# bacpop/ska.rust

Hardware: AMD Instinct MI355X
Metric: genomes/sec ska build+align, 1 000x5 Mbp k=31; bit-exact vs CPU (higher is better)
Workload: dtype u64

## Files before the change

### ska.rust_amd/csrc/skx_api.cpp

```cpp
#include "skx_internal.h"
#include "../../include/skx_host.h"
#include <algorithm>
#include <atomic>
#include <chrono>
#include <cmath>
#include <cstdarg>
#include <cstddef>
#include <cstdio>
#include <cstring>
#include <map>
#include <memory>
#include <mutex>
#include <numeric>
#include <optional>
#include <unordered_map>
#include <thread>
#include <cerrno>
#include <fcntl.h>
#include <sys/mman.h>
#include <sys/stat.h>
#include <unistd.h>

using namespace skx;

// ... 1115 lines not shown
    }
    SKX_HIP(hipStreamSynchronize(st));
    *out = a.release();
    return SKX_OK;
}
static int lazy_check_missing(skx_array *a, DevBuf<int> &d_flag)
{
    int missing = 0;
    SKX_HIP(hipMemcpyAsync(&missing, d_flag.p, 4, hipMemcpyDeviceToHost, a->ctx->stream));
    SKX_HIP(hipStreamSynchronize(a->ctx->stream));
    SKX_HIP(hipGetLastError());
    if (missing) { set_error("row keyset does not contain every split k-mer of the samples"); return SKX_EINVAL; }
    return SKX_OK;
}
extern "C" int skx_array_assemble_lazy(skx_ctx *ctx, skx_dictset *d, skx_keyset *rows, const char *const *names, skx_array **out)
{
    return skx_guarded([&]() -> int {
    if (!ctx || !d || !rows || !out) { skx_dictset_free(d); skx_keyset_free(rows); set_error("bad arguments"); return SKX_EINVAL; }
    if (rows->holds_pieces_of(d)) {
        const int r = skx_array_assemble(ctx, d, rows, names, out);
        skx_dictset_free(d); skx_keyset_free(rows);
        return r;
    }
    if (rows->wide != d->wide() || rows->k != d->k || rows->rc != d->rc || rows->logN < 0 || rows->logN < d->logB || d->n > 65535 || knob("eager_array")) {
        const int r = skx_array_assemble(ctx, d, rows, names, out);
        skx_dictset_free(d); skx_keyset_free(rows);
        return r;
    }
    SKX_HIP(hipSetDevice(ctx->device));
    { const int rs = dictset_sort(d); if (rs != SKX_OK) { skx_dictset_free(d); skx_keyset_free(rows); return rs; } }
    return array_make_lazy(ctx, d, rows, names, out);
    });
}
static int pieces_stats_pass(skx_array *a, uint64_t min_count)
{
    skx_ctx *ctx = a->ctx; hipStream_t st = ctx->stream;
    const skx_pieces *pc = a->pieces; const skx_keyset *blk = a->lazy_rows;
    const int S = (int)a->names.size(), nb = 1 << pc->logQ;
    ctx->cut_ranks = ctx->cut_blocks = 0;
    if (!a->n_rows) return SKX_OK;
    const uint32_t stage = min_count >= 2 ? pieces_stats_bound(pc->cap) : 0u;
    DevBuf<uint32_t> r_cut; DevBuf<unsigned long long> tally;
    if (stage) { SKX_TRY(r_cut.alloc((size_t)nb)); SKX_TRY(tally.alloc(2)); SKX_TRY(tally.zero(st)); }
    unsigned long long h_tally[2] = {0, 0};
    {
        StageTimer t(ctx, &ctx->tm.assemble);
        KernelTimer kt(ctx, &ctx->tm.pieces_stats);
        if (stage) launch_pieces_cut(pc->plen.p, S, pc->cap, (uint32_t)std::min<uint64_t>(min_count, 0xFFFFFFFEull), pc->nrank.p, blk->ncnt.p, stage, nb, r_cut.p, tally.p, st);
        launch_pieces_stats(pc->data.p, pc->plen.p, pc->perm.p, pc->nrank.p, blk->ncnt.p, blk->roff.p, pc->cap, S, nb, a->present.p, a->unambig.p, a->mask.p, a->vcount.p, st,
                            stage ? r_cut.p : nullptr);
        if (stage) SKX_HIP(hipMemcpyAsync(h_tally, tally.p, 16, hipMemcpyDeviceToHost, st));
    }
    SKX_HIP(hipStreamSynchronize(st));
    SKX_HIP(hipGetLastError());
    ctx->cut_ranks = h_tally[0]; ctx->cut_blocks = h_tally[1];
    if (stage && getenv("SKX_DEBUG")) fprintf(stderr, "[skx] filter: min_count %llu, the rank bound left %llu ranks unread over %llu of %d row blocks\n", (unsigned long long)min_count, h_tally[0], h_tally[1], nb);
    return SKX_OK;
}
int skx::array_lazy_stats(skx_array *a)
{
    if (!a->lazy() || a->stats_ready) return SKX_OK;
    skx_ctx *ctx = a->ctx; hipStream_t st = ctx->stream;
    SKX_HIP(hipSetDevice(ctx->device));
    if (a->pieces) {
        SKX_TRY(pieces_stats_pass(a, 0));
        a->stats_ready = true;
        return SKX_OK;
    }
    DevBuf<int> d_flag; SKX_TRY(d_flag.alloc(1)); SKX_TRY(d_flag.zero(st));
    if (a->n_rows) {
        AssembleArgs aa = lazy_args(a, d_flag.p);
        { StageTimer t(ctx, &ctx->tm.assemble); launch_assemble_lazy(a, aa, st, 1); }
        SKX_HIP(hipMemcpyAsync(a->vcount.p, a->present.p, a->n_rows * 4, hipMemcpyDeviceToDevice, st));
    }
    SKX_TRY(lazy_check_missing(a, d_flag));
    a->stats_ready = true;
    return SKX_OK;
}
int skx::array_materialize(skx_array *a)
{
    if (!a->lazy()) return SKX_OK;
    skx_ctx *ctx = a->ctx; hipStream_t st = ctx->stream;
    SKX_HIP(hipSetDevice(ctx->device));
    if (a->pieces) SKX_TRY(array_lazy_stats(a));
    const uint64_t U = a->n_rows; const size_t S = a->names.size();
    a->pitch = pitch_for(U);
    SKX_TRY(a->matrix.alloc((uint64_t)S * a->pitch));
    DevBuf<int> d_flag; SKX_TRY(d_flag.alloc(1)); SKX_TRY(d_flag.zero(st));
    if (a->pieces) {
// ... 560 lines not shown
                launch_compact_u64(a->keys.p, k2.p, U, keep.p, pos.p, st);
                a->keys = std::move(k2);
            } else if (a->host_keys.empty()) {
                DevBuf<uint64_t> k2; SKX_TRY(k2.alloc(kept * 2));
                launch_compact_u128(a->keys.p, k2.p, U, keep.p, pos.p, st);
                a->keys = std::move(k2);
            } else {
                std::vector<uint8_t> hkeep(U);
                SKX_HIP(hipMemcpyAsync(hkeep.data(), keep.p, U, hipMemcpyDeviceToHost, st));
                SKX_HIP(hipStreamSynchronize(st));
                std::vector<skx_key> nk; nk.reserve(kept);
                for (uint64_t i = 0; i < U; i++) if (hkeep[i] == 1) nk.push_back(a->host_keys[i]);
                a->host_keys.swap(nk);
            }
            a->n_kmers = kept;
        }
        SKX_HIP(hipStreamSynchronize(st));
        a->matrix = std::move(nm); a->present = std::move(p2); a->unambig = std::move(u2); a->mask = std::move(m2); a->vcount = std::move(v2);
        a->pitch = np; a->n_rows = kept;
        a->drop_lazy();
        a->stats_ready = true;
    }
    return SKX_OK;
}

extern "C" int skx_array_filter(skx_array *a, uint64_t min_count, int filter_ambig_as_missing, int filter_type, int mask_ambig,
                                int ignore_const_gaps, int update_kmers, int32_t *removed)
{
    return skx_guarded([&]() -> int {
    skx_ctx *ctx = a->ctx; hipStream_t st = ctx->stream;
    SKX_HIP(hipSetDevice(ctx->device));
    const uint64_t U = a->n_rows; const size_t S = a->names.size();
    ctx->cut_ranks = ctx->cut_blocks = 0;
    if (a->pieces && !a->stats_ready && !filter_ambig_as_missing && min_count >= 2 && a->total_samples == 0 && !knob("stats_eager"))
        SKX_TRY(pieces_stats_pass(a, min_count));
    else
        SKX_TRY(array_lazy_stats(a));
    DevBuf<uint8_t> keep; DevBuf<uint64_t> pos;
    SKX_TRY(keep.alloc(U)); SKX_TRY(pos.alloc(U + 1));
    uint64_t kept = 0, silent = 0;
    {
        StageTimer t(ctx, &ctx->tm.filter);
        FilterArgs fa{a->vcount.p, a->present.p, a->unambig.p, a->mask.p, U, (uint32_t)(a->total_samples ? a->total_samples : S), min_count, filter_ambig_as_missing, filter_type, ignore_const_gaps, keep.p};
        launch_filter_flags(fa, st);
        DevBuf<uint32_t> sc_sums; DevBuf<uint64_t> sc_offs;
        SKX_TRY(sc_sums.alloc(scan_u8_blocks(U))); SKX_TRY(sc_offs.alloc(scan_u8_blocks(U) + 1));
        launch_scan_u8(keep.p, pos.p, U, sc_sums.p, sc_offs.p, st);
        SKX_HIP(hipMemcpyAsync(&kept, pos.p + U, 8, hipMemcpyDeviceToHost, st));
        if (filter_ambig_as_missing) {
            DevBuf<unsigned long long> d_sil; SKX_TRY(d_sil.alloc(1)); SKX_TRY(d_sil.zero(st));
            launch_count_u8(keep.p, U, 2, d_sil.p, st);
            unsigned long long s2 = 0;
            SKX_HIP(hipMemcpyAsync(&s2, d_sil.p, 8, hipMemcpyDeviceToHost, st));
            SKX_HIP(hipStreamSynchronize(st));
            silent = s2;
        }
        SKX_HIP(hipStreamSynchronize(st));
    }
    SKX_TRY(array_compact(a, keep, pos, kept, mask_ambig, filter_ambig_as_missing != 0, update_kmers || filter_ambig_as_missing));
    SKX_HIP(hipGetLastError());
    if (removed) *removed = (int32_t)(U - kept - silent);
    return SKX_OK;
    });
}


static int array_keep_rows(skx_array *a, DevBuf<uint8_t> &keep, uint64_t *removed)
{
    hipStream_t st = a->ctx->stream;
    const uint64_t U = a->n_rows;
    DevBuf<uint64_t> pos; SKX_TRY(pos.alloc(U + 1));
    uint64_t kept = 0;
    DevBuf<uint32_t> sc_sums; DevBuf<uint64_t> sc_offs;
    SKX_TRY(sc_sums.alloc(scan_u8_blocks(U))); SKX_TRY(sc_offs.alloc(scan_u8_blocks(U) + 1));
    launch_scan_u8(keep.p, pos.p, U, sc_sums.p, sc_offs.p, st);
    SKX_HIP(hipMemcpyAsync(&kept, pos.p + U, 8, hipMemcpyDeviceToHost, st));
    SKX_HIP(hipStreamSynchronize(st));
    SKX_TRY(array_compact(a, keep, pos, kept, 0, false, true));
    SKX_HIP(hipGetLastError());
    if (removed) *removed = U - kept;
    return SKX_OK;
}

extern "C" skx_ctx *skx_array_ctx(const skx_array *a) { return a->ctx; }
extern "C" void skx_set_last_error(const char *msg) { set_error("%s", msg ? msg : ""); }

extern "C" int skx_keyset_from_fasta(skx_ctx *ctx, const char *path, int k, int rc, skx_keyset **out)
{
    return skx_guarded([&]() -> int {
    if (!ctx || !path || !out) { set_error("bad arguments"); return SKX_EINVAL; }
    SKX_TRY(check_k(k));
// ... 335 lines not shown
```

### ska.rust_amd/csrc/skx_append.hip

```cpp
#include "skx_device.h"
#include <cstdlib>
#include <type_traits>

namespace skx {

typedef uint32_t u32x4 __attribute__((ext_vector_type(4)));
typedef const u32x4 __attribute__((address_space(1))) *g4_t;

#ifdef SKX_AP_PROF
__device__ unsigned long long g_ap_prof[16];
#define AP_PROF_START unsigned long long tprof = __builtin_readcyclecounter(), tacc[12] = {0, 0, 0, 0, 0, 0, 0, 0, 0, 0, 0, 0}
#define AP_PROF(i) do { const unsigned long long t_ = __builtin_readcyclecounter(); tacc[(i)] += t_ - tprof; tprof = t_; } while (0)
#define AP_PROF_FLUSH() do { for (int i_ = 0; i_ < 12; i_++) if (tacc[i_] && (i_ >= 6 || (threadIdx.x & 63) == 0)) atomicAdd(&g_ap_prof[i_], tacc[i_]); } while (0)
extern "C" void skx_debug_phase_prof(unsigned long long *out, int reset)
{
    unsigned long long h[16];
    (void)hipDeviceSynchronize();
    (void)hipMemcpyFromSymbol(h, HIP_SYMBOL(g_ap_prof), sizeof(h));
    for (int i = 0; i < 16; i++) out[i] = h[i];
    if (reset) { for (auto &x : h) x = 0; (void)hipMemcpyToSymbol(HIP_SYMBOL(g_ap_prof), h, sizeof(h)); }
}
#else
#define AP_PROF_START do { } while (0)
#define AP_PROF(i) do { } while (0)
// ... 426 lines not shown
        }
    }
    __syncthreads();
    uint16_t *pj = a.perm + j * (uint64_t)cap;
    for (uint32_t i = tid; i < cap; i += AP_THREADS) pj[i] = s_perm[i];
    if (tid == 0) { a.ncnt[j] = total; a.nrank[j] = nr < cap ? nr : cap; if (total > a.stride) atomicOr(a.overflow, 1); }
    __syncthreads();
    }
}

template <bool COUNT_ONLY>
static void launch_append_t(const AppendArgs &a, unsigned blocks, hipStream_t st)
{
    const size_t lds = append_lds_bytes(a.nslots, a.cap, COUNT_ONLY);
    const bool hi = a.bits - a.logQ >= 32;
    if (hi) {
        (void)hipFuncSetAttribute((const void *)append_kernel<COUNT_ONLY, true>, hipFuncAttributeMaxDynamicSharedMemorySize, (int)lds);
        hipLaunchKernelGGL((append_kernel<COUNT_ONLY, true>), dim3(blocks), dim3(AP_THREADS), lds, st, a);
    } else {
        (void)hipFuncSetAttribute((const void *)append_kernel<COUNT_ONLY, false>, hipFuncAttributeMaxDynamicSharedMemorySize, (int)lds);
        hipLaunchKernelGGL((append_kernel<COUNT_ONLY, false>), dim3(blocks), dim3(AP_THREADS), lds, st, a);
    }
}
bool append_ok(int bits, int logB, int logQ, uint32_t region_cap, uint32_t nslots, uint32_t cap)
{
    const int rem = bits - logQ;
    (void)region_cap;
    return logQ >= logB && rem >= 0 && rem <= 50 && cap % 128u == 0 && cap >= 128u && cap <= APPEND_MAX_CAP && nslots >= cap && (nslots & (nslots - 1u)) == 0u &&
           append_lds_bytes(nslots, cap, false) <= 160u * 1024u - 256u;
}
void launch_append(const AppendArgs &a, uint32_t region_cap, hipStream_t st) { (void)region_cap; launch_append_t<false>(a, (1u << a.logQ) / a.rounds, st); }
void launch_append_probe(const AppendArgs &a, uint32_t region_cap, unsigned blocks, hipStream_t st) { (void)region_cap; launch_append_t<true>(a, blocks, st); }

__global__ __launch_bounds__(256) void pieces_cut_kernel(const uint16_t *plen, int S, uint32_t cap, uint32_t min_count, const uint32_t *nrank, const uint32_t *ncnt,
                                                         uint32_t stage, uint32_t *r_cut, unsigned long long *tally)
{
    extern __shared__ uint32_t s_hist[];
    __shared__ uint32_t s_sum[256];
    __shared__ uint32_t s_cut;
    const uint64_t j = blockIdx.x;
    const uint32_t tid = threadIdx.x, nbin = cap + 1u, share = (nbin + 255u) / 256u;
    for (uint32_t i = tid; i < nbin; i += 256) s_hist[i] = 0;
    if (tid == 0) s_cut = 0;
    __syncthreads();
    const uint16_t *pl = plen + j * (uint64_t)S;
    for (int s = (int)tid; s < S; s += 256) { const uint32_t v = pl[s]; atomicAdd(&s_hist[v < cap ? v : cap], 1u); }
    __syncthreads();
    const uint32_t b0 = tid * share, b1 = b0 + share < nbin ? b0 + share : nbin;
    uint32_t own = 0;
    for (uint32_t b = b0; b < b1; b++) own += s_hist[b];
    s_sum[tid] = own;
    __syncthreads();
    uint32_t above = 0;
    for (uint32_t t = tid + 1; t < 256; t++) above += s_sum[t];
    if (min_count >= 1u && above < min_count && min_count <= above + own) {
        uint32_t acc = above;
        for (uint32_t b = b1; b-- > b0;) { acc += s_hist[b]; if (acc >= min_count) { s_cut = b; break; } }
    }
    __syncthreads();
    if (tid == 0) {
        uint32_t rc = min_count ? s_cut : 0xFFFFFFFFu;
        if (ncnt && ncnt[j] > stage) rc = 0xFFFFFFFFu;
        r_cut[j] = rc;
        if (tally && nrank) {
            const uint32_t nr = nrank[j], lim = nr < rc ? nr : rc;
            const uint64_t seen = (uint64_t)((lim + 31u) / 32u) * 32u;
            if (seen < nr) { atomicAdd(&tally[0], (unsigned long long)(nr - seen)); atomicAdd(&tally[1], 1ull); }
        }
    }
}
void launch_pieces_cut(const uint16_t *plen, int n_samples, uint32_t cap, uint32_t min_count, const uint32_t *nrank, const uint32_t *ncnt, uint32_t stage, int n_blocks,
                       uint32_t *r_cut, unsigned long long *tally, hipStream_t st)
{
    if (n_blocks <= 0) return;
    hipLaunchKernelGGL(pieces_cut_kernel, dim3((unsigned)n_blocks), dim3(256), ((size_t)cap + 1) * 4, st, plen, n_samples, cap, min_count, nrank, ncnt, stage, r_cut, tally);
}

__global__ __launch_bounds__(256) void pieces_stats_kernel(const uint8_t *pieces, const uint16_t *plen, const uint16_t *perm, const uint32_t *nrank, const uint32_t *ncnt,
                                                           const uint64_t *roff, uint32_t cap, int S, uint32_t *o_present, uint32_t *o_unambig, uint32_t *o_mask,
                                                           uint32_t *o_vcount, int force_direct, uint32_t stage, const uint32_t *r_cut)
{
    constexpr int W = 4;
    extern __shared__ __attribute__((aligned(16))) uint16_t s_stage[];
    const uint32_t PS_STAGE = stage;
    uint16_t *const s_pr = s_stage, *const s_un = s_stage + stage, *const s_mk = s_stage + 2 * (size_t)stage;
    const uint64_t j = blockIdx.x;
    const uint32_t nr = nrank[j], nrows = ncnt[j];
    const uint64_t r0 = roff[j];
    const uint32_t d = blockIdx.y * 256u + threadIdx.x;
    if (blockIdx.y * 256u * 8u * W >= nr && !(blockIdx.y == 0 && nrows)) return;
    const bool staged = gridDim.y == 1 && nrows <= PS_STAGE && !force_direct;
    if (staged) {
        for (uint32_t p = threadIdx.x; p < nrows; p += 256) { s_pr[p] = 0; s_un[p] = 0; s_mk[p] = 0; }
        __syncthreads();
    }
    const int lane = threadIdx.x & 63, wv = threadIdx.x >> 6;
    const uint16_t *pl = plen + j * (uint64_t)S;
    const uint4 *col = reinterpret_cast<const uint4 *>(pieces + j * (uint64_t)S * (cap / 2)) + d;
    const uint32_t step = cap / 32;
    uint32_t lim = nr;
    if (r_cut && staged) { const uint32_t rc = r_cut[j]; if (rc < lim) lim = rc; }
    const uint32_t nseen = (lim + 31u) / 32u * 32u < nr ? (lim + 31u) / 32u * 32u : nr;
    const bool mine = d * 32u < lim;
    const bool wave_has = (d - (uint32_t)(threadIdx.x & 63)) * 32u < lim;
    uint32_t pN[W], aN[W];
    uint32_t pE[W], pO[W], aE[W], aO[W], uni[W];
    uint32_t PE0[W], PE1[W], PO0[W], PO1[W], AE0[W], AE1[W], AO0[W], AO1[W];
#pragma unroll
    for (int w = 0; w < W; w++) { pN[w] = aN[w] = 0; pE[w] = pO[w] = aE[w] = aO[w] = uni[w] = 0; PE0[w] = PE1[w] = PO0[w] = PO1[w] = AE0[w] = AE1[w] = AO0[w] = AO1[w] = 0; }
    auto nibfold = [&]() {
#pragma unroll
        for (int w = 0; w < W; w++) {
            pE[w] += pN[w] & 0x0F0F0F0Fu; pO[w] += (pN[w] >> 4) & 0x0F0F0F0Fu; aE[w] += aN[w] & 0x0F0F0F0Fu; aO[w] += (aN[w] >> 4) & 0x0F0F0F0Fu;
            pN[w] = aN[w] = 0;
        }
    };
    auto fold = [&]() {
        nibfold();
#pragma unroll
        for (int w = 0; w < W; w++) {
            PE0[w] += pE[w] & 0x00FF00FFu; PE1[w] += (pE[w] >> 8) & 0x00FF00FFu; PO0[w] += pO[w] & 0x00FF00FFu; PO1[w] += (pO[w] >> 8) & 0x00FF00FFu;
            AE0[w] += aE[w] & 0x00FF00FFu; AE1[w] += (aE[w] >> 8) & 0x00FF00FFu; AO0[w] += aO[w] & 0x00FF00FFu; AO1[w] += (aO[w] >> 8) & 0x00FF00FFu;
            pE[w] = pO[w] = aE[w] = aO[w] = 0;
        }
    };
    auto take = [&](int w, uint32_t x) {
        uint32_t t = x | (x >> 1); t |= t >> 2;
        const uint32_t nz = t & 0x11111111u;
        const uint32_t y = x & (x - nz);
        uint32_t u = y | (y >> 1); u |= u >> 2;
        const uint32_t am = u & 0x11111111u;
        pN[w] += nz; aN[w] += am;
        uni[w] |= x;
    };
    for (int s0 = 0, since = 0, nib = 0; wave_has && s0 < S; s0 += 64) {
        const uint32_t plv = s0 + lane < S ? (uint32_t)pl[s0 + lane] : 0u;
        const int n = S - s0 < 64 ? S - s0 : 64;
#pragma unroll 1
        for (int i0 = 0; i0 < n; i0 += 4) {
            if (nib == 12) { nibfold(); nib = 0; }
            nib += 4;
            uint4 x[4];
#pragma unroll
            for (int u = 0; u < 4; u++) {
                const uint32_t l = (uint32_t)__builtin_amdgcn_readlane((int)plv, (i0 + u) & 63);
                x[u] = make_uint4(0u, 0u, 0u, 0u);
                if (mine && i0 + u < n && d * 32u < l) x[u] = col[(uint64_t)(s0 + i0 + u) * step];
            }
#pragma unroll
            for (int u = 0; u < 4; u++) { take(0, x[u].x); take(1, x[u].y); take(2, x[u].z); take(3, x[u].w); }
        }
        since += 64;
        if (since >= 192) { fold(); since = 0; nib = 0; }
    }
    fold();
    const uint16_t *pj = perm + j * (uint64_t)cap;
    if (mine) {
#pragma unroll
        for (int w = 0; w < W; w++) {
            uint32_t pres[8], amb[8];
            pres[0] = PE0[w] & 0xFFFFu; pres[4] = PE0[w] >> 16; pres[2] = PE1[w] & 0xFFFFu; pres[6] = PE1[w] >> 16;
            pres[1] = PO0[w] & 0xFFFFu; pres[5] = PO0[w] >> 16; pres[3] = PO1[w] & 0xFFFFu; pres[7] = PO1[w] >> 16;
            amb[0] = AE0[w] & 0xFFFFu; amb[4] = AE0[w] >> 16; amb[2] = AE1[w] & 0xFFFFu; amb[6] = AE1[w] >> 16;
            amb[1] = AO0[w] & 0xFFFFu; amb[5] = AO0[w] >> 16; amb[3] = AO1[w] & 0xFFFFu; amb[7] = AO1[w] >> 16;
            const uint4 pv = *reinterpret_cast<const uint4 *>(pj + d * 32u + (uint32_t)w * 8u);
            const uint32_t pw[4] = {pv.x, pv.y, pv.z, pv.w};
#pragma unroll
            for (int i = 0; i < 8; i++) {
                const uint32_t r = d * 32u + (uint32_t)w * 8u + i;
                if (r >= nr) break;
                const uint32_t p = (pw[i >> 1] >> (16 * (i & 1))) & 0xFFFFu;
                if (p >= nrows) continue;
                const uint32_t u = (uni[w] >> (4 * i)) & 15u;
                const uint32_t mk = ((u & 1u) << 1) | ((u & 2u) << 1) | ((u & 4u) << 2) | ((u & 8u) << 5);
                if (staged) { s_pr[p] = (uint16_t)pres[i]; s_un[p] = (uint16_t)(pres[i] - amb[i]); s_mk[p] = (uint16_t)mk; }
                else {
                    o_vcount[r0 + p] = pres[i];
                    __hip_atomic_store(&o_present[r0 + p], pres[i], __ATOMIC_RELAXED, __HIP_MEMORY_SCOPE_AGENT);
                    __hip_atomic_store(&o_unambig[r0 + p], pres[i] - amb[i], __ATOMIC_RELAXED, __HIP_MEMORY_SCOPE_AGENT);
                    o_mask[r0 + p] = mk;
                }
            }
        }
    }
    if (!staged) __threadfence();
    __syncthreads();
    const uint32_t rk0 = blockIdx.y * 256u * 8u * W, rk1 = rk0 + 256u * 8u * W < nseen ? rk0 + 256u * 8u * W : nseen;
    for (uint32_t rb = rk0 + (uint32_t)wv * 64u; rb < rk1; rb += 256u) {
// ... 10 lines not shown
        while (todo) {
            const int src = __builtin_ctzll(todo);
            todo &= todo - 1;
            const uint32_t r = rb + (uint32_t)src, prow = (uint32_t)__shfl((int)pp, src, 64);
            uint32_t m = 0;
            for (int t = lane; t < S; t += 64) {
                if ((uint32_t)pl[t] <= r) continue;
                const uint32_t x = *(reinterpret_cast<const uint32_t *>(pieces + (j * (uint64_t)S + t) * (cap / 2)) + (r >> 3));
                const uint32_t nib = (x >> ((r & 7u) * 4u)) & 15u;
                if (nib) m |= 1u << nib;
            }
#pragma unroll
            for (int dd = 32; dd >= 1; dd >>= 1) m |= __shfl_xor(m, dd, 64);
            if (lane == 0) { if (staged) s_mk[prow] = (uint16_t)m; else o_mask[r0 + prow] = m; }
        }
    }
    if (!staged) return;
    __syncthreads();
    for (uint32_t p = threadIdx.x; p < nrows; p += 256) {
        const uint32_t pr = s_pr[p];
        o_present[r0 + p] = pr; o_vcount[r0 + p] = pr;
        o_unambig[r0 + p] = s_un[p]; o_mask[r0 + p] = s_mk[p];
    }
}
namespace {
struct StatsLaunch { unsigned gy; int direct; uint32_t stage; bool bounded() const { return gy == 1 && !direct; } };
StatsLaunch stats_launch(uint32_t cap)
{
    static const int direct = knob("stats_direct") ? 1 : 0;
    return {(cap / 32 + 255u) / 256u, direct, (cap + 63u) / 64u * 64u};
}
}
void launch_pieces_stats(const uint8_t *pieces, const uint16_t *plen, const uint16_t *perm, const uint32_t *nrank, const uint32_t *ncnt, const uint64_t *roff, uint32_t cap,
                         int n_samples, int n_blocks, uint32_t *present, uint32_t *unambig, uint32_t *mask, uint32_t *vcount, hipStream_t st, const uint32_t *r_cut)
{
    if (n_blocks <= 0) return;
    const StatsLaunch l = stats_launch(cap);
    if (!l.bounded()) r_cut = nullptr;
    hipLaunchKernelGGL(pieces_stats_kernel, dim3((unsigned)n_blocks, l.gy), dim3(256), (size_t)l.stage * 6, st, pieces, plen, perm, nrank, ncnt, roff, cap, n_samples, present, unambig, mask, vcount,
                       l.direct, l.stage, r_cut);
}
uint32_t pieces_stats_bound(uint32_t cap) { const StatsLaunch l = stats_launch(cap); return l.bounded() ? l.stage : 0u; }
__global__ __launch_bounds__(256) void pieces_cells_kernel(const uint8_t *pieces, const uint16_t *plen, uint32_t cap, int S, unsigned long long *out)
{
    const uint64_t j = blockIdx.x;
    const int lane = threadIdx.x & 63;
    for (int s = blockIdx.y * 4 + (threadIdx.x >> 6); s < S; s += gridDim.y * 4) {
        const uint32_t pl = plen[j * (uint64_t)S + s];
        const uint32_t *src = reinterpret_cast<const uint32_t *>(pieces + (j * (uint64_t)S + s) * (cap / 2));
        uint32_t c = 0;
        for (uint32_t i = lane; i < (pl + 7u) / 8u; i += 64) { const uint32_t x = src[i]; uint32_t t = x | (x >> 1); t |= t >> 2; c += (uint32_t)__popc(t & 0x11111111u); }
#pragma unroll
        for (int dd = 32; dd >= 1; dd >>= 1) c += __shfl_xor(c, dd, 64);
        if (lane == 0 && c) atomicAdd(&out[s], (unsigned long long)c);
    }
}
void launch_pieces_cells(const uint8_t *pieces, const uint16_t *plen, uint32_t cap, int n_samples, int n_blocks, unsigned long long *out, hipStream_t st)
{
    if (n_blocks <= 0 || n_samples <= 0) return;
    unsigned gy = (unsigned)((n_samples + 3) / 4); if (gy > 16) gy = 16;
    hipLaunchKernelGGL(pieces_cells_kernel, dim3((unsigned)n_blocks, gy), dim3(256), 0, st, pieces, plen, cap, n_samples, out);
}
__global__ __launch_bounds__(256) void region_totals_kernel(const uint32_t *raw, int logB, unsigned long long *out)
{
    __shared__ unsigned long long s_sum[256];
    const uint64_t B = 1ull << logB;
    unsigned long long t = 0;
    for (uint64_t b = threadIdx.x; b < B; b += 256) t += raw[(uint64_t)blockIdx.x * B + b];
    s_sum[threadIdx.x] = t;
    __syncthreads();
    for (int d = 128; d >= 1; d >>= 1) { if ((int)threadIdx.x < d) s_sum[threadIdx.x] += s_sum[threadIdx.x + d]; __syncthreads(); }
    if (threadIdx.x == 0) out[blockIdx.x] = s_sum[0];
}
void launch_region_totals(const uint32_t *raw, int n_samples, int logB, unsigned long long *out, hipStream_t st)
{
    if (n_samples > 0) hipLaunchKernelGGL(region_totals_kernel, dim3((unsigned)n_samples), dim3(256), 0, st, raw, logB, out);
}

constexpr int PR_WAVES = 8;
__device__ static inline uint32_t ap_iupac4(uint32_t m)
{
    const uint32_t idx = m & 0x07070707u;
    const uint32_t lo = __builtin_amdgcn_perm(0x48595754u, 0x4D43412Du, idx);
    const uint32_t hi = __builtin_amdgcn_perm(0x4E42444Bu, 0x56535247u, idx);
    const uint32_t sel = ((m >> 3) & 0x01010101u) * 0xFFu;
    return (hi & sel) | (lo & ~sel);
}
template <bool KEPT>
__global__ __launch_bounds__(64 * PR_WAVES) void pieces_rows_kernel(PiecesRowsArgs a)
{
    extern __shared__ __attribute__((aligned(16))) unsigned char s_raw[];
    const uint32_t cap = a.cap;
    uint16_t *s_src = reinterpret_cast<uint16_t *>(s_raw);
    uint32_t *s_piece = reinterpret_cast<uint32_t *>(s_raw + (((size_t)cap + 16) * 2 + 15) / 16 * 16);
    const uint64_t j = (uint64_t)blockIdx.x + a.j_base;
    const uint32_t n = a.ncnt[j];
    if (n == 0) return;
    const uint64_t r0 = a.roff[j];
    const uint64_t k0 = KEPT ? a.kpos[r0] : 0;
    const uint32_t nout = KEPT ? (uint32_t)(a.kpos[r0 + n] - k0) : n;
    if (nout == 0) return;
    const int tid = threadIdx.x, lane = tid & 63, wv = tid >> 6;
    const uint64_t ocol = KEPT ? k0 : r0 - a.col_base;
    const uint32_t shift = (uint32_t)(ocol & 3u);
    const uint32_t ndw = (nout + shift + 3u) / 4u;
    const uint16_t *pj = a.perm + j * (uint64_t)cap;
    const uint32_t nr = a.nrank[j];
    const int S = a.n_samples;
    const int s_lo = blockIdx.y * a.samples_per_wg, s_hi = s_lo + a.samples_per_wg < S ? s_lo + a.samples_per_wg : S;
    uint32_t *pc = s_piece + (size_t)wv * (cap / 8 + 4);
    const unsigned char *pcb = reinterpret_cast<const unsigned char *>(pc);
    __shared__ uint32_t s_top;
    uint32_t nrw = (nr + 7u) / 8u;
    if (lane < 4) pc[cap / 8 + lane] = 0u;
    for (uint32_t t0 = 0; t0 < nout + shift; t0 += cap) {
        for (uint32_t i = tid; i < cap + 16u; i += blockDim.x) s_src[i] = (uint16_t)cap;
        if (KEPT && tid == 0) s_top = 0;
        __syncthreads();
        uint32_t top = 0;
        for (uint32_t r = tid; r < nr; r += blockDim.x) {
            const uint32_t p = pj[r];
            if (p == 0xFFFFu || p >= n) continue;
            uint32_t sc;
            if (!KEPT) sc = shift + p;
            else if (a.keep[r0 + p] == 1) sc = shift + (uint32_t)(a.kpos[r0 + p] - k0);
            else continue;
            if (sc >= t0 && sc < t0 + cap) { s_src[sc - t0] = (uint16_t)r; top = r + 1u; }
        }
        if (KEPT && top) atomicMax(&s_top, top);
        __syncthreads();
        if (KEPT && !a.full_pieces) nrw = (s_top + 7u) / 8u;
        const uint32_t v_lo = t0 / 4u, v_hi = (t0 + cap) / 4u < ndw ? (t0 + cap) / 4u : ndw;
        for (int s = s_lo + wv; s < s_hi; s += PR_WAVES) {
            const uint32_t pl = a.plen[j * (uint64_t)S + s];
            const uint32_t plw = (pl + 7u) / 8u;
            const uint32_t *src = reinterpret_cast<const uint32_t *>(a.pieces + (j * (uint64_t)S + s) * (cap / 2));
            {
                const uint4 *src4 = reinterpret_cast<const uint4 *>(src);
                uint4 *pc4 = reinterpret_cast<uint4 *>(pc);
                for (uint32_t i = lane; i < (nrw + 3u) / 4u; i += 64) {
                    uint4 x = 4u * i < plw ? src4[i] : make_uint4(0u, 0u, 0u, 0u);
                    if (4u * i + 1u >= plw) x.y = 0u;
                    if (4u * i + 2u >= plw) x.z = 0u;
                    if (4u * i + 3u >= plw) x.w = 0u;
                    pc4[i] = x;
                }
            }
            __builtin_amdgcn_wave_barrier();
            unsigned char *dst = a.out + (uint64_t)s * a.pitch + (ocol - shift);
            for (uint32_t v = v_lo + lane; v < v_hi; v += 64) {
                const uint2 rr = *reinterpret_cast<const uint2 *>(s_src + 4u * (v - v_lo));
                const uint32_t ra = rr.x & 0xFFFFu, rb = rr.x >> 16, rc = rr.y & 0xFFFFu, rd = rr.y >> 16;
                const uint32_t na = ((uint32_t)pcb[ra >> 1] >> ((ra & 1u) * 4u)) & 15u, nb = ((uint32_t)pcb[rb >> 1] >> ((rb & 1u) * 4u)) & 15u;
                const uint32_t nc = ((uint32_t)pcb[rc >> 1] >> ((rc & 1u) * 4u)) & 15u, nd = ((uint32_t)pcb[rd >> 1] >> ((rd & 1u) * 4u)) & 15u;
                uint32_t m = na | (nb << 8) | (nc << 16) | (nd << 24);
                uint32_t word = ap_iupac4(m);
                if (a.mask_ambig) {
                    const uint32_t y = m & (m - ((m | (m >> 1) | (m >> 2) | (m >> 3)) & 0x01010101u));
                    const uint32_t amb = ((y | (y >> 1) | (y >> 2) | (y >> 3)) & 0x01010101u) * 0xFFu;
                    word = (word & ~amb) | (0x4E4E4E4Eu & amb);
                }
                const bool head = v == 0 && shift != 0, tail = v == ndw - 1 && ((nout + shift) & 3u) != 0;
                if (!head && !tail) *reinterpret_cast<uint32_t *>(dst + 4u * v) = word;
                else {
#pragma unroll
                    for (int b = 0; b < 4; b++) { const int c = (int)(4u * v + b) - (int)shift; if (c >= 0 && (uint32_t)c < nout) dst[4u * v + b] = (unsigned char)(word >> (8 * b)); }
                }
            }
            __builtin_amdgcn_wave_barrier();
        }
        __syncthreads();
    }
}
void launch_pieces_rows(const PiecesRowsArgs &a, uint32_t n_blocks, hipStream_t st)
{
    if (!n_blocks || a.n_samples <= 0) return;
    PiecesRowsArgs b = a;
    int spw = a.n_samples;
    while (spw > PR_WAVES * 4 && (uint64_t)n_blocks * ((a.n_samples + spw - 1) / spw) < 8192) spw = (spw + 1) / 2;
    b.samples_per_wg = spw;
    const unsigned gy = (unsigned)((a.n_samples + spw - 1) / spw);
// ... 14 lines not shown
```

### ska.rust_amd/csrc/skx_device.h

```cpp
#pragma once
#include <hip/hip_runtime.h>
#include <stdint.h>

namespace skx {

long knob(const char *name, long absent = 0);
int extract_tile_bases(int logB);
constexpr int MAX_LOGB = 13;
constexpr uint64_t EMPTY64 = ~0ull;

struct HashParams {
    int bits;
    int hb;
    uint32_t hmask;
    uint32_t c[4];
};
HashParams make_hash_params(int k);
__host__ __device__ inline uint32_t hround(uint32_t v, uint32_t c, int hb) { return (v * c) >> (32 - hb); }
__host__ __device__ inline void hmix_halves(uint32_t &L, uint32_t &R, const HashParams &p)
{
    L ^= hround(R, p.c[0], p.hb); R ^= hround(L, p.c[1], p.hb);
}
__host__ __device__ inline uint64_t hmix(uint64_t x, const HashParams &p)
{
// ... 94 lines not shown
    int mask_ambig = 0;
};
void launch_assemble(const AssembleArgs &a, hipStream_t st, int mode = 0, uint32_t n_blocks = 0);
bool union_side_ok(const DictView &d, int logN, uint32_t stride);
void launch_union_side(const DictView &d, int logN, uint64_t *stage, uint32_t stride, uint32_t *ncnt, uint32_t table_slots, int *overflow,
                       uint16_t *side, uint16_t *perm, hipStream_t st);
void launch_assemble_side(const AssembleArgs &a, const uint16_t *side, const uint16_t *perm, hipStream_t st, bool wide = false);
void launch_compose_perm(const uint64_t *l_stage, uint32_t l_stride, const uint32_t *l_ncnt, const uint16_t *l_perm, int l_logN, const uint64_t *g_stage,
                         uint32_t g_stride, const uint32_t *g_ncnt, const uint64_t *g_roff, int g_logN, int bits, uint16_t *g_perm, uint32_t *g_n,
                         uint64_t *g_base, uint32_t *g_max, int *bad, hipStream_t st);
void launch_union_side_wide(const DictView &d, int logN, u128 *stage, uint32_t stride, uint32_t *ncnt, uint32_t table_slots, int *overflow,
                            uint16_t *side, uint16_t *perm, hipStream_t st);

constexpr uint32_t APPEND_MAX_CAP = 6016, APPEND_MAX_SLOTS = 8192;
struct AppendArgs {
    const uint64_t *words; const uint64_t *off; const uint32_t *raw;
    int n_samples, logB, bits, logQ;
    uint32_t nslots, cap;
    uint8_t *pieces; uint16_t *plen; uint16_t *perm; uint32_t *nrank;
    uint64_t *stage; uint32_t stride; uint32_t *ncnt;
    unsigned long long *probe;
    int *overflow;
    uint32_t rounds = 1;
    int *bar = nullptr;
};
bool append_ok(int bits, int logB, int logQ, uint32_t region_cap, uint32_t nslots, uint32_t cap);
void launch_append(const AppendArgs &a, uint32_t region_cap, hipStream_t st);
void launch_append_probe(const AppendArgs &a, uint32_t region_cap, unsigned blocks, hipStream_t st);
constexpr uint32_t APPEND_WIDE_MAX_CAP = 3072, APPEND_WIDE_MAX_SLOTS = 4096;
bool append_wide_ok(int bits, int logB, int logQ, uint32_t nslots, uint32_t cap);
void launch_append_wide(const AppendArgs &a, hipStream_t st);
void launch_append_wide_probe(const AppendArgs &a, unsigned blocks, hipStream_t st);
void launch_pieces_stats(const uint8_t *pieces, const uint16_t *plen, const uint16_t *perm, const uint32_t *nrank, const uint32_t *ncnt, const uint64_t *roff, uint32_t cap,
                         int n_samples, int n_blocks, uint32_t *present, uint32_t *unambig, uint32_t *mask, uint32_t *vcount, hipStream_t st, const uint32_t *r_cut = nullptr);
void launch_pieces_cut(const uint16_t *plen, int n_samples, uint32_t cap, uint32_t min_count, const uint32_t *nrank, const uint32_t *ncnt, uint32_t stage, int n_blocks,
                       uint32_t *r_cut, unsigned long long *tally, hipStream_t st);
uint32_t pieces_stats_bound(uint32_t cap);
void launch_pieces_cells(const uint8_t *pieces, const uint16_t *plen, uint32_t cap, int n_samples, int n_blocks, unsigned long long *out, hipStream_t st);
void launch_region_totals(const uint32_t *raw, int n_samples, int logB, unsigned long long *out, hipStream_t st);
struct PiecesRowsArgs {
    const uint8_t *pieces; const uint16_t *plen; const uint16_t *perm; const uint32_t *nrank; uint32_t cap; int n_samples;
    const uint32_t *ncnt; const uint64_t *roff;
    uint8_t *out; uint64_t pitch;
    uint32_t j_base = 0; uint64_t col_base = 0;
    const uint8_t *keep = nullptr; const uint64_t *kpos = nullptr;
    int mask_ambig = 0;
    int full_pieces = 0;
    int samples_per_wg = 0;
};
void launch_pieces_rows(const PiecesRowsArgs &a, uint32_t n_blocks, hipStream_t st);

void launch_gather_keys(const uint64_t *stage, uint32_t stride, const uint32_t *ncnt, const uint64_t *roff, int n_sub,
                        uint64_t *out, int unhash, HashParams hp, hipStream_t st);
void launch_hash_keys(const uint64_t *keys, uint64_t *words, uint64_t n, HashParams hp, hipStream_t st);
void launch_keys_cbor(const uint64_t *words, uint64_t n, HashParams hp, uint8_t *out, int *short_key, hipStream_t st);
void launch_unhash_dict(const uint64_t *words, uint64_t n, uint64_t *keys, uint8_t *bases, HashParams hp, hipStream_t st);

void launch_col_stats(const uint8_t *matrix, uint64_t pitch, int n_samples, uint64_t n_cols, uint32_t *present,
                      uint32_t *unambig, uint32_t *mask, int *bad_byte, hipStream_t st);
struct FilterArgs {
    const uint32_t *vcount, *present, *unambig, *mask; uint64_t n_cols; uint32_t n_samples;
    uint64_t min_count; int ambig_as_missing, filter_type, ignore_const_gaps;
    uint8_t *keep;
    int two_stage = 0;
};
void launch_filter_flags(const FilterArgs &a, hipStream_t st);
void launch_row_stats_rm(const uint8_t *cells, uint64_t S, uint64_t nr, uint32_t *present, uint32_t *unambig, uint32_t *mask, int *bad_byte, hipStream_t st);
// ... 109 lines not shown
```

Before: 29480.

## Fuse rank-cut into stats kernel, split samples across waves, prefetch piece rows

The separate pieces_cut kernel is folded into pieces_stats: each block computes its rank cut in shared memory, using a wave-shuffle scan in place of a serial suffix sum. This drops one launch and the r_cut buffer, and the tally readback moves into the filter's existing sync, removing a host synchronisation. When few columns are active, stats now splits the sample loop across idle waves and reduces their partial counts through shared memory. The pieces_rows copy loop gains register prefetch of the next sample's piece data. Together these add complexity and extra syncthreads, and increase shared-memory reuse risk.

```diff
diff --git a/ska.rust_amd/csrc/skx_api.cpp b/ska.rust_amd/csrc/skx_api.cpp
--- a/ska.rust_amd/csrc/skx_api.cpp
+++ b/ska.rust_amd/csrc/skx_api.cpp
@@ -1171,29 +1171,23 @@
     return array_make_lazy(ctx, d, rows, names, out);
     });
 }
-static int pieces_stats_pass(skx_array *a, uint64_t min_count)
+static int pieces_stats_pass(skx_array *a, uint64_t min_count, DevBuf<unsigned long long> *tally = nullptr)
 {
     skx_ctx *ctx = a->ctx; hipStream_t st = ctx->stream;
     const skx_pieces *pc = a->pieces; const skx_keyset *blk = a->lazy_rows;
     const int S = (int)a->names.size(), nb = 1 << pc->logQ;
     ctx->cut_ranks = ctx->cut_blocks = 0;
     if (!a->n_rows) return SKX_OK;
-    const uint32_t stage = min_count >= 2 ? pieces_stats_bound(pc->cap) : 0u;
-    DevBuf<uint32_t> r_cut; DevBuf<unsigned long long> tally;
-    if (stage) { SKX_TRY(r_cut.alloc((size_t)nb)); SKX_TRY(tally.alloc(2)); SKX_TRY(tally.zero(st)); }
-    unsigned long long h_tally[2] = {0, 0};
+    const bool bounded = min_count >= 2 && tally && pieces_stats_bound(pc->cap);
+    if (bounded) { SKX_TRY(tally->alloc(2)); SKX_TRY(tally->zero(st)); }
     {
         StageTimer t(ctx, &ctx->tm.assemble);
         KernelTimer kt(ctx, &ctx->tm.pieces_stats);
-        if (stage) launch_pieces_cut(pc->plen.p, S, pc->cap, (uint32_t)std::min<uint64_t>(min_count, 0xFFFFFFFEull), pc->nrank.p, blk->ncnt.p, stage, nb, r_cut.p, tally.p, st);
         launch_pieces_stats(pc->data.p, pc->plen.p, pc->perm.p, pc->nrank.p, blk->ncnt.p, blk->roff.p, pc->cap, S, nb, a->present.p, a->unambig.p, a->mask.p, a->vcount.p, st,
-                            stage ? r_cut.p : nullptr);
-        if (stage) SKX_HIP(hipMemcpyAsync(h_tally, tally.p, 16, hipMemcpyDeviceToHost, st));
-    }
-    SKX_HIP(hipStreamSynchronize(st));
+                            bounded ? (uint32_t)std::min<uint64_t>(min_count, 0xFFFFFFFEull) : 0u, bounded ? tally->p : nullptr);
+    }
+    if (!bounded) SKX_HIP(hipStreamSynchronize(st));
     SKX_HIP(hipGetLastError());
-    ctx->cut_ranks = h_tally[0]; ctx->cut_blocks = h_tally[1];
-    if (stage && getenv("SKX_DEBUG")) fprintf(stderr, "[skx] filter: min_count %llu, the rank bound left %llu ranks unread over %llu of %d row blocks\n", (unsigned long long)min_count, h_tally[0], h_tally[1], nb);
     return SKX_OK;
 }
 int skx::array_lazy_stats(skx_array *a)
@@ -1820,8 +1814,10 @@
     SKX_HIP(hipSetDevice(ctx->device));
     const uint64_t U = a->n_rows; const size_t S = a->names.size();
     ctx->cut_ranks = ctx->cut_blocks = 0;
+    DevBuf<unsigned long long> tally;
+    unsigned long long h_tally[2] = {0, 0};
     if (a->pieces && !a->stats_ready && !filter_ambig_as_missing && min_count >= 2 && a->total_samples == 0 && !knob("stats_eager"))
-        SKX_TRY(pieces_stats_pass(a, min_count));
+        SKX_TRY(pieces_stats_pass(a, min_count, &tally));
     else
         SKX_TRY(array_lazy_stats(a));
     DevBuf<uint8_t> keep; DevBuf<uint64_t> pos;
@@ -1835,6 +1831,7 @@
         SKX_TRY(sc_sums.alloc(scan_u8_blocks(U))); SKX_TRY(sc_offs.alloc(scan_u8_blocks(U) + 1));
         launch_scan_u8(keep.p, pos.p, U, sc_sums.p, sc_offs.p, st);
         SKX_HIP(hipMemcpyAsync(&kept, pos.p + U, 8, hipMemcpyDeviceToHost, st));
+        if (tally.p) SKX_HIP(hipMemcpyAsync(h_tally, tally.p, 16, hipMemcpyDeviceToHost, st));
         if (filter_ambig_as_missing) {
             DevBuf<unsigned long long> d_sil; SKX_TRY(d_sil.alloc(1)); SKX_TRY(d_sil.zero(st));
             launch_count_u8(keep.p, U, 2, d_sil.p, st);
@@ -1845,6 +1842,8 @@
         }
         SKX_HIP(hipStreamSynchronize(st));
     }
+    ctx->cut_ranks = h_tally[0]; ctx->cut_blocks = h_tally[1];
+    if (tally.p && getenv("SKX_DEBUG")) fprintf(stderr, "[skx] filter: min_count %llu, the rank bound left %llu ranks unread over %llu of %d row blocks\n", (unsigned long long)min_count, h_tally[0], h_tally[1], 1 << a->pieces->logQ);
     SKX_TRY(array_compact(a, keep, pos, kept, mask_ambig, filter_ambig_as_missing != 0, update_kmers || filter_ambig_as_missing));
     SKX_HIP(hipGetLastError());
     if (removed) *removed = (int32_t)(U - kept - silent);
diff --git a/ska.rust_amd/csrc/skx_append.hip b/ska.rust_amd/csrc/skx_append.hip
--- a/ska.rust_amd/csrc/skx_append.hip
+++ b/ska.rust_amd/csrc/skx_append.hip
@@ -482,41 +482,52 @@
 void launch_append(const AppendArgs &a, uint32_t region_cap, hipStream_t st) { (void)region_cap; launch_append_t<false>(a, (1u << a.logQ) / a.rounds, st); }
 void launch_append_probe(const AppendArgs &a, uint32_t region_cap, unsigned blocks, hipStream_t st) { (void)region_cap; launch_append_t<true>(a, blocks, st); }
 
-__global__ __launch_bounds__(256) void pieces_cut_kernel(const uint16_t *plen, int S, uint32_t cap, uint32_t min_count, const uint32_t *nrank, const uint32_t *ncnt,
-                                                         uint32_t stage, uint32_t *r_cut, unsigned long long *tally)
-{
-    extern __shared__ uint32_t s_hist[];
-    __shared__ uint32_t s_sum[256];
+__device__ static inline uint32_t pieces_cut_block(const uint16_t *pl, int S, uint32_t cap, uint32_t min_count, uint32_t *s_hist)
+{
+    __shared__ uint32_t s_wave[4];
     __shared__ uint32_t s_cut;
-    const uint64_t j = blockIdx.x;
-    const uint32_t tid = threadIdx.x, nbin = cap + 1u, share = (nbin + 255u) / 256u;
+    const uint32_t tid = threadIdx.x, lane = tid & 63u, wv = tid >> 6, nbin = cap + 1u, share = (nbin + 255u) / 256u;
     for (uint32_t i = tid; i < nbin; i += 256) s_hist[i] = 0;
     if (tid == 0) s_cut = 0;
     __syncthreads();
-    const uint16_t *pl = plen + j * (uint64_t)S;
     for (int s = (int)tid; s < S; s += 256) { const uint32_t v = pl[s]; atomicAdd(&s_hist[v < cap ? v : cap], 1u); }
     __syncthreads();
-    const uint32_t b0 = tid * share, b1 = b0 + share < nbin ? b0 + share : nbin;
+    const uint32_t b0 = tid * share < nbin ? tid * share : nbin, b1 = b0 + share < nbin ? b0 + share : nbin;
     uint32_t own = 0;
     for (uint32_t b = b0; b < b1; b++) own += s_hist[b];
-    s_sum[tid] = own;
-    __syncthreads();
-    uint32_t above = 0;
-    for (uint32_t t = tid + 1; t < 256; t++) above += s_sum[t];
+    uint32_t incl = own;
+#pragma unroll
+    for (int dd = 1; dd < 64; dd <<= 1) { const uint32_t o = (uint32_t)__shfl_down((int)incl, dd, 64); if (lane + (uint32_t)dd < 64u) incl += o; }
+    if (lane == 0) s_wave[wv] = incl;
+    __syncthreads();
+    uint32_t above = incl - own;
+    for (uint32_t w = wv + 1; w < 4; w++) above += s_wave[w];
     if (min_count >= 1u && above < min_count && min_count <= above + own) {
         uint32_t acc = above;
         for (uint32_t b = b1; b-- > b0;) { acc += s_hist[b]; if (acc >= min_count) { s_cut = b; break; } }
     }
     __syncthreads();
-    if (tid == 0) {
-        uint32_t rc = min_count ? s_cut : 0xFFFFFFFFu;
+    const uint32_t rc = s_cut;
+    __syncthreads();
+    return rc;
+}
+__device__ static inline void pieces_cut_tally(uint32_t nr, uint32_t rc, unsigned long long *tally)
+{
+    const uint32_t lim = nr < rc ? nr : rc;
+    const uint64_t seen = (uint64_t)((lim + 31u) / 32u) * 32u;
+    if (seen < nr) { atomicAdd(&tally[0], (unsigned long long)(nr - seen)); atomicAdd(&tally[1], 1ull); }
+}
+__global__ __launch_bounds__(256) void pieces_cut_kernel(const uint16_t *plen, int S, uint32_t cap, uint32_t min_count, const uint32_t *nrank, const uint32_t *ncnt,
+                                                         uint32_t stage, uint32_t *r_cut, unsigned long long *tally)
+{
+    extern __shared__ uint32_t s_hist[];
+    const uint64_t j = blockIdx.x;
+    const uint32_t cut = pieces_cut_block(plen + j * (uint64_t)S, S, cap, min_count, s_hist);
+    if (threadIdx.x == 0) {
+        uint32_t rc = min_count ? cut : 0xFFFFFFFFu;
         if (ncnt && ncnt[j] > stage) rc = 0xFFFFFFFFu;
         r_cut[j] = rc;
-        if (tally && nrank) {
-            const uint32_t nr = nrank[j], lim = nr < rc ? nr : rc;
-            const uint64_t seen = (uint64_t)((lim + 31u) / 32u) * 32u;
-            if (seen < nr) { atomicAdd(&tally[0], (unsigned long long)(nr - seen)); atomicAdd(&tally[1], 1ull); }
-        }
+        if (tally && nrank) pieces_cut_tally(nrank[j], rc, tally);
     }
 }
 void launch_pieces_cut(const uint16_t *plen, int n_samples, uint32_t cap, uint32_t min_count, const uint32_t *nrank, const uint32_t *ncnt, uint32_t stage, int n_blocks,
@@ -528,7 +539,7 @@
 
 __global__ __launch_bounds__(256) void pieces_stats_kernel(const uint8_t *pieces, const uint16_t *plen, const uint16_t *perm, const uint32_t *nrank, const uint32_t *ncnt,
                                                            const uint64_t *roff, uint32_t cap, int S, uint32_t *o_present, uint32_t *o_unambig, uint32_t *o_mask,
-                                                           uint32_t *o_vcount, int force_direct, uint32_t stage, const uint32_t *r_cut)
+                                                           uint32_t *o_vcount, int force_direct, uint32_t stage, uint32_t min_count, unsigned long long *tally)
 {
     constexpr int W = 4;
     extern __shared__ __attribute__((aligned(16))) uint16_t s_stage[];
@@ -537,22 +548,29 @@
     const uint64_t j = blockIdx.x;
     const uint32_t nr = nrank[j], nrows = ncnt[j];
     const uint64_t r0 = roff[j];
-    const uint32_t d = blockIdx.y * 256u + threadIdx.x;
     if (blockIdx.y * 256u * 8u * W >= nr && !(blockIdx.y == 0 && nrows)) return;
     const bool staged = gridDim.y == 1 && nrows <= PS_STAGE && !force_direct;
-    if (staged) {
-        for (uint32_t p = threadIdx.x; p < nrows; p += 256) { s_pr[p] = 0; s_un[p] = 0; s_mk[p] = 0; }
-        __syncthreads();
-    }
-    const int lane = threadIdx.x & 63, wv = threadIdx.x >> 6;
+    const int lane = threadIdx.x & 63, wv = __builtin_amdgcn_readfirstlane((int)(threadIdx.x >> 6));
     const uint16_t *pl = plen + j * (uint64_t)S;
+    uint32_t lim = nr;
+    if (min_count && staged) {
+        const uint32_t rc = pieces_cut_block(pl, S, cap, min_count, reinterpret_cast<uint32_t *>(s_stage));
+        if (threadIdx.x == 0 && tally) pieces_cut_tally(nr, rc, tally);
+        if (rc < lim) lim = rc;
+    }
+    const uint32_t nseen = (lim + 31u) / 32u * 32u < nr ? (lim + 31u) / 32u * 32u : nr;
+    const uint32_t ncol = (lim + 31u) / 32u, ncg = ncol < 64u ? ncol : 64u;
+    uint32_t G = 4, P = 1;
+    if (staged && ncol) {
+        G = (ncol + 63u) / 64u;
+        for (P = 4u / G; P > 1u && (P / 2u) * G * 36u * 4u * ncg > PS_STAGE * 6u; P >>= 1) { }
+    }
+    const uint32_t grp = (uint32_t)wv % G, slice = (uint32_t)wv / G;
+    const uint32_t d = blockIdx.y * 256u + grp * 64u + (uint32_t)lane;
     const uint4 *col = reinterpret_cast<const uint4 *>(pieces + j * (uint64_t)S * (cap / 2)) + d;
     const uint32_t step = cap / 32;
-    uint32_t lim = nr;
-    if (r_cut && staged) { const uint32_t rc = r_cut[j]; if (rc < lim) lim = rc; }
-    const uint32_t nseen = (lim + 31u) / 32u * 32u < nr ? (lim + 31u) / 32u * 32u : nr;
-    const bool mine = d * 32u < lim;
-    const bool wave_has = (d - (uint32_t)(threadIdx.x & 63)) * 32u < lim;
+    bool mine = slice < P && d * 32u < lim;
+    const bool wave_has = slice < P && (d - (uint32_t)lane) * 32u < lim;
     uint32_t pN[W], aN[W];
     uint32_t pE[W], pO[W], aE[W], aO[W], uni[W];
     uint32_t PE0[W], PE1[W], PO0[W], PO1[W], AE0[W], AE1[W], AO0[W], AO1[W];
@@ -583,7 +601,7 @@
         pN[w] += nz; aN[w] += am;
         uni[w] |= x;
     };
-    for (int s0 = 0, since = 0, nib = 0; wave_has && s0 < S; s0 += 64) {
+    for (int s0 = (int)slice * 64, since = 0, nib = 0; wave_has && s0 < S; s0 += 64 * (int)P) {
         const uint32_t plv = s0 + lane < S ? (uint32_t)pl[s0 + lane] : 0u;
         const int n = S - s0 < 64 ? S - s0 : 64;
 #pragma unroll 1
@@ -604,6 +622,36 @@
         if (since >= 192) { fold(); since = 0; nib = 0; }
     }
     fold();
+    if (P > 1u) {
+        uint32_t *const xch = reinterpret_cast<uint32_t *>(s_stage);
+        for (uint32_t half = P >> 1; half >= 1u; half >>= 1) {
+            if (mine && slice >= half && slice < 2u * half) {
+                uint32_t *const xa = xch + ((size_t)((slice - half) * G + grp) * 36u) * ncg + (uint32_t)lane;
+#pragma unroll
+                for (int w = 0; w < W; w++) {
+                    uint32_t *q = xa + (size_t)w * 9u * ncg;
+                    q[0] = PE0[w]; q[ncg] = PE1[w]; q[2 * ncg] = PO0[w]; q[3 * ncg] = PO1[w]; q[4 * ncg] = AE0[w]; q[5 * ncg] = AE1[w]; q[6 * ncg] = AO0[w]; q[7 * ncg] = AO1[w];
+                    q[8 * ncg] = uni[w];
+                }
+            }
+            __syncthreads();
+            if (mine && slice < half) {
+                const uint32_t *const xb = xch + ((size_t)(slice * G + grp) * 36u) * ncg + (uint32_t)lane;
+#pragma unroll
+                for (int w = 0; w < W; w++) {
+                    const uint32_t *q = xb + (size_t)w * 9u * ncg;
+                    PE0[w] += q[0]; PE1[w] += q[ncg]; PO0[w] += q[2 * ncg]; PO1[w] += q[3 * ncg]; AE0[w] += q[4 * ncg]; AE1[w] += q[5 * ncg]; AO0[w] += q[6 * ncg]; AO1[w] += q[7 * ncg];
+                    uni[w] |= q[8 * ncg];
+                }
+            }
+            __syncthreads();
+        }
+        if (slice) mine = false;
+    }
+    if (staged) {
+        for (uint32_t p = threadIdx.x; p < nrows; p += 256) { s_pr[p] = 0; s_un[p] = 0; s_mk[p] = 0; }
+        __syncthreads();
+    }
     const uint16_t *pj = perm + j * (uint64_t)cap;
     if (mine) {
 #pragma unroll
@@ -680,13 +728,13 @@
 }
 }
 void launch_pieces_stats(const uint8_t *pieces, const uint16_t *plen, const uint16_t *perm, const uint32_t *nrank, const uint32_t *ncnt, const uint64_t *roff, uint32_t cap,
-                         int n_samples, int n_blocks, uint32_t *present, uint32_t *unambig, uint32_t *mask, uint32_t *vcount, hipStream_t st, const uint32_t *r_cut)
+                         int n_samples, int n_blocks, uint32_t *present, uint32_t *unambig, uint32_t *mask, uint32_t *vcount, hipStream_t st, uint32_t min_count, unsigned long long *tally)
 {
     if (n_blocks <= 0) return;
     const StatsLaunch l = stats_launch(cap);
-    if (!l.bounded()) r_cut = nullptr;
+    if (!l.bounded()) min_count = 0;
     hipLaunchKernelGGL(pieces_stats_kernel, dim3((unsigned)n_blocks, l.gy), dim3(256), (size_t)l.stage * 6, st, pieces, plen, perm, nrank, ncnt, roff, cap, n_samples, present, unambig, mask, vcount,
-                       l.direct, l.stage, r_cut);
+                       l.direct, l.stage, min_count, tally);
 }
 uint32_t pieces_stats_bound(uint32_t cap) { const StatsLaunch l = stats_launch(cap); return l.bounded() ? l.stage : 0u; }
 __global__ __launch_bounds__(256) void pieces_cells_kernel(const uint8_t *pieces, const uint16_t *plen, uint32_t cap, int S, unsigned long long *out)
@@ -726,6 +774,7 @@
 }
 
 constexpr int PR_WAVES = 8;
+constexpr int PR_AHEAD = 3;
 __device__ static inline uint32_t ap_iupac4(uint32_t m)
 {
     const uint32_t idx = m & 0x07070707u;
@@ -779,22 +828,40 @@
         __syncthreads();
         if (KEPT && !a.full_pieces) nrw = (s_top + 7u) / 8u;
         const uint32_t v_lo = t0 / 4u, v_hi = (t0 + cap) / 4u < ndw ? (t0 + cap) / 4u : ndw;
-        for (int s = s_lo + wv; s < s_hi; s += PR_WAVES) {
-            const uint32_t pl = a.plen[j * (uint64_t)S + s];
-            const uint32_t plw = (pl + 7u) / 8u;
-            const uint32_t *src = reinterpret_cast<const uint32_t *>(a.pieces + (j * (uint64_t)S + s) * (cap / 2));
-            {
-                const uint4 *src4 = reinterpret_cast<const uint4 *>(src);
-                uint4 *pc4 = reinterpret_cast<uint4 *>(pc);
-                for (uint32_t i = lane; i < (nrw + 3u) / 4u; i += 64) {
-                    uint4 x = 4u * i < plw ? src4[i] : make_uint4(0u, 0u, 0u, 0u);
-                    if (4u * i + 1u >= plw) x.y = 0u;
-                    if (4u * i + 2u >= plw) x.z = 0u;
-                    if (4u * i + 3u >= plw) x.w = 0u;
-                    pc4[i] = x;
-                }
+        const int cnt = __builtin_amdgcn_readfirstlane(s_lo + wv < s_hi ? (s_hi - s_lo - wv + PR_WAVES - 1) / PR_WAVES : 0);
+        const uint32_t n4 = (nrw + 3u) / 4u;
+        const uint16_t *plj = a.plen + j * (uint64_t)S + s_lo + wv;
+        uint4 *pc4 = reinterpret_cast<uint4 *>(pc);
+        auto masked = [&](uint4 x, uint32_t i, uint32_t plw) {
+            if (4u * i >= plw) x.x = 0u;
+            if (4u * i + 1u >= plw) x.y = 0u;
+            if (4u * i + 2u >= plw) x.z = 0u;
+            if (4u * i + 3u >= plw) x.w = 0u;
+            return x;
+        };
+        uint32_t plv = 0, plw = 0, plw_next = 0;
+        uint4 nx[PR_AHEAD];
+#pragma unroll
+        for (int u = 0; u < PR_AHEAD; u++) nx[u] = make_uint4(0u, 0u, 0u, 0u);
+        auto ask = [&](int i) {
+            if ((i & 63) == 0) plv = i + lane < cnt ? (uint32_t)plj[(size_t)(i + lane) * PR_WAVES] : 0u;
+            plw_next = ((uint32_t)__builtin_amdgcn_readlane((int)plv, i & 63) + 7u) / 8u;
+            const uint4 *src4 = reinterpret_cast<const uint4 *>(a.pieces + (j * (uint64_t)S + (uint64_t)(s_lo + wv + i * PR_WAVES)) * (cap / 2));
+#pragma unroll
+            for (int u = 0; u < PR_AHEAD; u++) { const uint32_t i4 = (uint32_t)lane + 64u * u; if (i4 < n4 && 4u * i4 < plw_next) nx[u] = src4[i4]; }
+        };
+        if (cnt > 0) ask(0);
+        for (int it = 0; it < cnt; it++) {
+            const int s = s_lo + wv + it * PR_WAVES;
+            plw = plw_next;
+#pragma unroll
+            for (int u = 0; u < PR_AHEAD; u++) { const uint32_t i4 = (uint32_t)lane + 64u * u; if (i4 < n4) pc4[i4] = masked(nx[u], i4, plw); }
+            if (n4 > 64u * PR_AHEAD) {
+                const uint4 *src4 = reinterpret_cast<const uint4 *>(a.pieces + (j * (uint64_t)S + (uint64_t)s) * (cap / 2));
+                for (uint32_t i4 = (uint32_t)lane + 64u * PR_AHEAD; i4 < n4; i4 += 64) pc4[i4] = masked(4u * i4 < plw ? src4[i4] : make_uint4(0u, 0u, 0u, 0u), i4, plw);
             }
             __builtin_amdgcn_wave_barrier();
+            if (it + 1 < cnt) ask(it + 1);
             unsigned char *dst = a.out + (uint64_t)s * a.pitch + (ocol - shift);
             for (uint32_t v = v_lo + lane; v < v_hi; v += 64) {
                 const uint2 rr = *reinterpret_cast<const uint2 *>(s_src + 4u * (v - v_lo));
diff --git a/ska.rust_amd/csrc/skx_device.h b/ska.rust_amd/csrc/skx_device.h
--- a/ska.rust_amd/csrc/skx_device.h
+++ b/ska.rust_amd/csrc/skx_device.h
@@ -150,7 +150,7 @@
 void launch_append_wide(const AppendArgs &a, hipStream_t st);
 void launch_append_wide_probe(const AppendArgs &a, unsigned blocks, hipStream_t st);
 void launch_pieces_stats(const uint8_t *pieces, const uint16_t *plen, const uint16_t *perm, const uint32_t *nrank, const uint32_t *ncnt, const uint64_t *roff, uint32_t cap,
-                         int n_samples, int n_blocks, uint32_t *present, uint32_t *unambig, uint32_t *mask, uint32_t *vcount, hipStream_t st, const uint32_t *r_cut = nullptr);
+                         int n_samples, int n_blocks, uint32_t *present, uint32_t *unambig, uint32_t *mask, uint32_t *vcount, hipStream_t st, uint32_t min_count = 0, unsigned long long *tally = nullptr);
 void launch_pieces_cut(const uint16_t *plen, int n_samples, uint32_t cap, uint32_t min_count, const uint32_t *nrank, const uint32_t *ncnt, uint32_t stage, int n_blocks,
                        uint32_t *r_cut, unsigned long long *tally, hipStream_t st);
 uint32_t pieces_stats_bound(uint32_t cap);
```

Result: faster. 30440 (median of 6 runs) (+3.3%).
